# yxtay/transformer-recommenders

Measured on AMD Instinct MI355X. Metric: user-sequences/sec (train step) MovieLens-1M seq200 d128 @1/2/4/8 GPU, higher is better.
Workload: dtype bf16; 1 GPU; MovieLens-1M-shaped: 3883 items, seq_len=200, d_model=128, 4-layer causal BERT (heads=4, ffn=512), InfoNCELoss over in-batch shared negatives, AdamW; per_gpu_batch=512, global_batch=512, seq_len=200, lengths=dense, loss_heads_evaluated=all 7 + LogitsStatistics (reference training_step), parallelism=dp1, launch=eager launches

## Files before the change

### include/xfmr_hip.h

```cpp
#ifndef XFMR_HIP_H
#define XFMR_HIP_H

#include <stddef.h>
#include <stdint.h>

#ifdef __cplusplus
extern "C" {
#endif

#define XFMR_ABI_VERSION 3

enum {
  XFMR_OK = 0,
  XFMR_EINVAL = -1,
  XFMR_EUNSUPPORTED = -2,
  XFMR_EWORKSPACE = -3,
  XFMR_EHIP = -4,
  XFMR_EALIGN = -5,
  XFMR_ECOMM = -6
};

enum { XFMR_PREC_F32 = 0, XFMR_PREC_BF16 = 1 };
enum { XFMR_ATTN_CAUSAL = 0, XFMR_ATTN_BIDIRECTIONAL = 1 };
enum { XFMR_ATTN_STREAM_KEYS = 2 };
// ... 159 lines not shown
typedef struct xfmr_loss_cfg {
  int32_t train_head;
  int32_t all_heads;
  int32_t mask_false_negatives;
  int32_t mode;
  int32_t precision;
  float scale;
  float margin;
  int32_t num_hard_negatives;
  uint32_t flags;
  void* profile_grad[2];
  void* profile_log[2];
  int64_t padded_positions;
} xfmr_loss_cfg;
enum {
  XFMR_LOSS_DTOK_ZEROED = 1u
};
#define XFMR_LOSS_NSPLIT(n) (((uint32_t)(n) & 0xffu) << 8)
#define XFMR_LOSS_NSPLIT_GRAD(n) (((uint32_t)(n) & 0xffu) << 16)
#define XFMR_LOSS_NSPLIT_OF(flags) (((flags) >> 8) & 0xffu)
#define XFMR_LOSS_NSPLIT_GRAD_OF(flags) (((flags) >> 16) & 0xffu)
size_t xfmr_sampled_loss_workspace(int64_t positions, int32_t H, int64_t n_rows);
size_t xfmr_sampled_loss_workspace_cfg(const xfmr_loss_cfg* cfg, int64_t positions, int32_t H, int64_t n_rows);
int xfmr_sampled_loss(const xfmr_loss_cfg* cfg, const float* tok, const uint8_t* key_mask, const int64_t* pos_idx,
                      const int64_t* neg_idx, const float* table, const float* table_rnorm, const void* table_bf16,
                      int64_t n_rows, int64_t positions, int32_t H, float* losses, float* stats, float* d_tok, void* workspace,
                      size_t workspace_bytes, void* stream);
size_t xfmr_sampled_loss_lists_workspace(int64_t n_query, int64_t n_neg, int32_t H, int64_t n_rows);
size_t xfmr_sampled_loss_lists_workspace_cfg(const xfmr_loss_cfg* cfg, int64_t n_query, int64_t n_neg, int32_t H,
                                             int64_t n_rows);
int xfmr_sampled_loss_lists(const xfmr_loss_cfg* cfg, const float* query, const int64_t* pos_items,
// ... 126 lines not shown
```

### transformer-recommenders_amd/csrc/internal.h

```cpp
#pragma once
#include "common.h"

enum : uint32_t {
  XF_S16_A = 1u,
  XF_S16_B = 2u,
  XF_S16_C = 4u,
  XF_S16_P = 8u,
  XF_AUX_GELU_GRAD = 0x100u,
};

enum GemmOp : int32_t {
  kGemmFwdBias = 0, kGemmFwdGelu, kGemmFwdDropRes,
  kGemmLnFwd, kGemmLnFwdRe, kGemmLnFwdReDrop,
  kGemmDx, kGemmDxGelu, kGemmDxLnBwd,
  kGemmDw, kGemmDwDeferred, kGemmDwGroup,
  kGemmFfnFwd, kGemmFfnFwdRe, kGemmFfnBwd,
  kGemmOps
};
enum GemmFamily : int32_t {
  kGemmNone = 0,
  kGemmTile,
  kGemmGroup,
  kGemmRing,
  kGemmFfnFwdKernel, kGemmFfnBwdKernel,
// ... 122 lines not shown
                       float* pre, float* mean, float* rstd, uint8_t* key_mask, int32_t B, int32_t L, int32_t H,
                       float eps, float dropout_p, XfSeed seed, uint32_t site, hipStream_t stream);
int xf_embed_ln_fwd_packed_ex(const int64_t* item_idx, const float* table, int64_t n_rows, const float* pos_emb,
                              const float* type_emb, const float* gamma, const float* beta, float* out, void* out16,
                              float* pre, float* mean, float* rstd, uint8_t* key_mask, int64_t rows, const int32_t* row_pos,
                              int32_t H, float eps, float dropout_p, XfSeed seed, uint32_t site, hipStream_t stream);
int xf_embed_param_grads_packed(const float* d_pre, float* d_pos, float* d_type, const int32_t* offs, int32_t B, int32_t L,
                                int32_t H, int32_t max_pos, hipStream_t st);
int xf_encoder_plan(const xfmr_encoder_cfg* cfg, int32_t out[16]);
int xf_attn_plan(int32_t bwd, int32_t precision, int32_t s16, int32_t B, int32_t L, int32_t A, int32_t H, int32_t causal,
                 int32_t packed, int32_t stream_keys, int32_t switches, int32_t out[8]);
int xf_attn_switches();
int xf_loss_plan(int64_t T, int32_t H, int64_t n_rows, int32_t train_head, int32_t all_heads, int32_t mask_false_negatives,
                 int32_t mode, int32_t precision, int32_t num_hard_negatives, uint32_t flags, int32_t has_d_tok,
                 int32_t has_table_bf16, int32_t cus, uint64_t switches, int32_t out[40]);
uint64_t xf_loss_switches();
int xf_layernorm_bwd_impl(const float* dy, const float* x, const float* mean, const float* rstd, const float* gamma,
                          float* dx, void* d_lin, bool lin16, float* d_gamma, float* d_beta, float* d_bias,
                          int64_t rows, int32_t H, XfDropout drop_out, XfDropout drop_lin, void* partials,
                          hipStream_t st, int* blocks_out = nullptr);
}
```

### transformer-recommenders_amd/csrc/loss.hip

```cpp
#include <stdlib.h>
#include <string.h>

#include "internal.h"
#include "loss_common.h"

namespace {

constexpr int PREP = 1024;
__global__ __launch_bounds__(PREP) void prepare_count_kernel(const uint8_t* key_mask, const int64_t* pos_idx, int T,
                                                             int2* blockcnt) {
  __shared__ int sv[PREP / 64], sq[PREP / 64];
  const int i = blockIdx.x * PREP + threadIdx.x;
  const bool v = i < T && key_mask[i] != 0;
  const bool q = v && pos_idx[i] != 0;
  const int nv = __popcll(__ballot(v)), nq = __popcll(__ballot(q));
  if ((threadIdx.x & 63) == 0) { sv[threadIdx.x >> 6] = nv; sq[threadIdx.x >> 6] = nq; }
  __syncthreads();
  if (threadIdx.x == 0) {
    int a = 0, b = 0;
    for (int w = 0; w < PREP / 64; ++w) { a += sv[w]; b += sq[w]; }
    blockcnt[blockIdx.x] = make_int2(a, b);
  }
}
__global__ __launch_bounds__(PREP) void prepare_write_kernel(const uint8_t* key_mask, const int64_t* pos_idx,
// ... 824 lines not shown
struct LossPass {
  int32_t role;
  int32_t code;
  int32_t all;
  int32_t gx, gy, gz;
  int32_t nsplit;
  int32_t buf;
  int32_t image;
  int32_t finish;
  int32_t pinned;
};
struct LossPlan {
  int32_t family, hard , qprep , npass;
  LossPass pass[2];
  int32_t need_grad, nsplit, nsplit_loss, loss_buf, lse_from_grad, skip_train_head, values_only, blocks;
};
constexpr int kLossPlanInts = sizeof(LossPlan) / sizeof(int32_t);

bool loss_key_ok(int64_t rows, int64_t n_rows, int train_head, int num_hard) {
  return rows > 0 && n_rows > 0 && rows <= (1 << 30) && n_rows <= (1 << 30) && train_head >= 0 &&
         train_head < XFMR_NUM_LOSSES && num_hard >= 0;
}
constexpr int loss_main_width(bool f32, int H) {
  if (H <= 0 || (H & 31)) return 0;
  for (int w : {64, 128, 256, 384, 512})
    if (H <= w) return w;
  if (f32) return 0;
  return H <= 768 ? 768 : H <= 1024 ? 1024 : 0;
}

int loss_plan(const LossKey& k, LossPlan& lp) {
  lp = LossPlan{};
// ... 48 lines not shown
    finish = grad_pass && ns_grad == 1 && !col_parts;
    const bool lse_elsewhere = head == XFMR_LOSS_INFONCE && (grad_pass || k.all_heads == 2);
    const int lcode = loss_dma_form(H, lse_elsewhere ? -2 : -1, mask_fn, k.mode, false, k.sw.logm256);
    auto add = [&](int role, int code, int gz, int n, int buf, bool fin) {
      const bool image = !k.sw.q_fp32 && n > 1;
      lp.qprep |= image;
      lp.pass[lp.npass++] = LossPass{role, code, 0, qblocks, n, gz, n, buf, image, fin, role == kPassGrad && pinned};
    };
    if (log_pass && pinned) add(kPassLog, lcode, 1, ns, 1, false);
    if (grad_pass) add(kPassGrad, gcode, parts, ns_grad, 0, finish);
    if (log_pass && !pinned) add(kPassLog, lcode, 1, ns, grad_pass, false);
    lp.nsplit = grad_pass ? ns_grad : ns;
    lp.loss_buf = grad_pass && log_pass;
    lp.nsplit_loss = lp.loss_buf ? ns : lp.nsplit;
    lp.lse_from_grad = lp.loss_buf && lse_elsewhere;
  }
  lp.need_grad = k.d_tok && !finish;
  lp.skip_train_head = k.all_heads == 2 && !k.d_tok;
  lp.values_only = !lp.need_grad;
  const int rows = lp.values_only ? kValueRows : kCombineRows;
  lp.blocks = (int)((k.T + rows - 1) / rows);
  return XFMR_OK;
}

template <class P, int W>
void launch_main(const LossArgs& a, bool all, dim3 grid, hipStream_t st) {
  if (all) hipLaunchKernelGGL((loss_main_kernel<P, W, true>), grid, dim3(256), 0, st, a);
  else hipLaunchKernelGGL((loss_main_kernel<P, W, false>), grid, dim3(256), 0, st, a);
}
template <class P>
// ... 47 lines not shown
                     losses, stats);
  XF_LAUNCH_CHECK();
  return XFMR_OK;
}

uint64_t xf_loss_switches() { return switch_bits(loss_switches()); }
int xf_loss_plan(int64_t T, int32_t H, int64_t n_rows, int32_t train_head, int32_t all_heads, int32_t mask_false_negatives,
                 int32_t mode, int32_t precision, int32_t num_hard_negatives, uint32_t flags, int32_t has_d_tok,
                 int32_t has_table_bf16, int32_t cus, uint64_t switches, int32_t out[40]) {
  static_assert(kLossPlanInts <= 40, "xf_loss_plan's array");
  LossPlan lp;
  const int rc = loss_plan(LossKey{T, n_rows, H, train_head, all_heads, mask_false_negatives, mode, precision,
                                   num_hard_negatives, flags, has_d_tok != 0, has_table_bf16 != 0, cus,
                                   switches_of(switches)}, lp);
  memset(out, 0, 40 * sizeof(int32_t));
  memcpy(out, &lp, sizeof(lp));
  return rc;
}

size_t xfmr_sampled_loss_workspace(int64_t positions, int32_t H, int64_t n_rows) {
  if (positions <= 0 || H <= 0) return 0;
  return loss_carve(nullptr, positions, H, n_rows).total;
}
size_t xfmr_sampled_loss_workspace_cfg(const xfmr_loss_cfg* cfg, int64_t positions, int32_t H, int64_t n_rows) {
  if (!cfg || positions <= 0 || H <= 0) return 0;
  return loss_carve(cfg, positions, H, n_rows).total;
}

static int run_loss(const xfmr_loss_cfg* cfg, const float* tok, const float* table, const float* table_rnorm,
                    const void* table_bf16, int64_t n_rows, int T, int32_t H, float* losses, float* stats, float* d_tok,
                    unsigned char* ws, const Plan& p, hipStream_t st) {
// ... 21 lines not shown
    if (int rc = launch_generic(d, lp.family, lp.pass[0].code, false, dim3(lp.pass[0].gx, lp.pass[0].gy), st)) return rc;
    SelectArgs s{};
    s.dump = d.dump; s.dump_ld = p.dump_ld; s.qinfo = d.qinfo; s.counts = counts; s.neg_item = neg_item;
    s.neg_rc = a.neg_rc; s.neg_mult = a.neg_mult; s.rnorm = table_rnorm; s.qpos = qpos; s.tau = (float4*)(ws + p.off_tau);
    s.mode = cfg->mode; s.mask_fn = cfg->mask_false_negatives; s.k = cfg->num_hard_negatives; s.n_rows = n_rows;
    hipLaunchKernelGGL(hard_select_kernel, dim3((unsigned)T), dim3(256), 0, st, s);
    XF_LAUNCH_CHECK();
    a.tau = (const float4*)(ws + p.off_tau);
  }
  bool img_ready = false;
  for (int i = 0; i < lp.npass; ++i) {
    const LossPass& ps = lp.pass[i];
    LossArgs l = a;
    l.nsplit = ps.nsplit; l.part = part[ps.buf];
    if (ps.role == kPassLog) l.need_grad = 0;
    if (ps.finish) l.d_tok = d_tok;
    if (ps.pinned) { l.pin_part = part[lp.loss_buf]; l.pin_nsplit = lp.nsplit_loss; }
    if (ps.image) {
      l.qimg = (__bf16*)(ws + p.off_qimg); l.qaux = (float2*)(ws + p.off_qaux);
      if (!img_ready) {
        if (int rc = launch_qprep_h(a, (__bf16*)(ws + p.off_qimg), (float2*)(ws + p.off_qaux), H, dim3(ps.gx), st)) return rc;
        img_ready = true;
      }
    }
    void* const* ev = ps.role == kPassGrad ? cfg->profile_grad : cfg->profile_log;
    if (ev[0] && hipEventRecord((hipEvent_t)ev[0], st) != hipSuccess) return XFMR_EHIP;
    const dim3 grid(ps.gx, ps.gy, ps.gz);
    if (int rc = lp.family == kLossDma ? launch_dma_h(l, table_bf16, H, ps.code, grid, st)
                                       : launch_generic(l, lp.family, ps.code, ps.all != 0, grid, st))
      return rc;
// ... 152 lines not shown
```

### transformer-recommenders_amd/csrc/loss_common.h

```cpp
#pragma once
#include "common.h"

namespace xfl {

constexpr int BN = 64;
constexpr int QB = 128;
constexpr int REC = 16;
constexpr int LDT = BN + 4;
constexpr float kLog2e = 1.4426950408889634f;
constexpr float kLn2 = 0.6931471805599453f;
enum { R_CNTD = 0, R_M, R_L, R_NCE, R_HINGE, R_LOGI, R_CNTC, R_CONTR, R_SSUM, R_SSQ, R_SMIN, R_SMAX, R_SW,
       R_POSDOT, R_RQ, R_QQ };
constexpr int BP = 24;
constexpr int HEAD_INFONCE_MASKED = XFMR_NUM_LOSSES;
constexpr int HEAD_INFONCE_PINNED = XFMR_NUM_LOSSES + 1;
constexpr int HEAD_BPR_MASKED = XFMR_NUM_LOSSES + 2;
constexpr int HEAD_CCL_MASKED = XFMR_NUM_LOSSES + 3, HEAD_CONTR_MASKED = XFMR_NUM_LOSSES + 4;

struct LossArgs {
  const float* tok; const float* table; const float* rnorm; int64_t n_rows;
  const int* counts;
  const int* neg_item;
  const float* neg_rc;
  const float* neg_mult;
  const int* qrow; const int* qpos;
  float* part; float* partO;
  float* dump; int64_t dump_ld; float2* qinfo; const float4* tau;
  const float* pin_part;
  int pin_nsplit;
  float* d_tok;
  const __bf16* qimg; const float2* qaux;
  int T; int nsplit;
  int H;
  int train_head, mask_fn, mode, need_grad;
  float scale, margin;
};

struct RowState {
  float cnt_d, m, l, nce, hinge, logi, cnt_c, contr, ssum, ssq, smin, smax, sw;
};
struct RowConst {
  float pos_dot, cpos, chinge, sc2, rq, margin;
  int pos_item, head;
  bool mask_fn, catalog, cos_head;
  bool hard;
  float tau_d, rho_d, tau_c, rho_c;
};
template <bool ALL, int HC, int NO, bool HARD = false>
__device__ __forceinline__ void loss_epilogue_t(f32x16& s, RowState& st, f32x16 (&o)[NO], const RowConst& k,
// ... 97 lines not shown
          w = d > 0.f ? mc * rc[u] : 0.f;
      }
      if (ALL) {
        ssum = fmaf(sv, md, ssum);
        ssq = fmaf(sv * sv, md, ssq);
        smin = fminf(smin, md > 0.f ? sv : INFINITY);
        smax = fmaxf(smax, md > 0.f ? sv : -INFINITY);
      }
      sw += w;
      s[r] = w;
    }
    __builtin_amdgcn_sched_barrier(0);
  }
}

template <bool CHECK_VALID>
__device__ __forceinline__ void loss_epilogue_infonce_masked(f32x16& s, float& l, float& cnt, float pos_dot, float sc2,
                                                             float m, int pos_item, const int* nid_sb,
                                                             const float* mu_sb, int hh) {
#pragma unroll
  for (int g = 0; g < 4; ++g) {
    const int4 n4 = *reinterpret_cast<const int4*>(&nid_sb[8 * g + 4 * hh]);
    const int nn[4] = {n4.x, n4.y, n4.z, n4.w};
    const float4 m4 = *reinterpret_cast<const float4*>(&mu_sb[8 * g + 4 * hh]);
    const float mu[4] = {m4.x, m4.y, m4.z, m4.w};
#pragma unroll
    for (int u = 0; u < 4; ++u) {
      const int r = 4 * g + u;
      bool counted = (s[r] < pos_dot) & (nn[u] != pos_item);
      if (CHECK_VALID) counted &= nn[u] >= 0;
      cnt += counted ? mu[u] : 0.f;
      const float e = xf_exp2(counted ? fmaf(s[r], sc2, -m) : -INFINITY) * mu[u];
      l += e;
      s[r] = e;
    }
  }
}

__device__ __forceinline__ void loss_epilogue_bpr_masked(f32x16& s, float& logi2, float& cnt, float& sw, float pos_dot,
                                                         float chinge, int pos_item, const int* nid_sb, const float* mu_sb,
                                                         int hh) {
#pragma unroll
  for (int g = 0; g < 4; ++g) {
    const int4 n4 = *reinterpret_cast<const int4*>(&nid_sb[8 * g + 4 * hh]);
    const int nn[4] = {n4.x, n4.y, n4.z, n4.w};
    const float4 m4 = *reinterpret_cast<const float4*>(&mu_sb[8 * g + 4 * hh]);
    const float mu[4] = {m4.x, m4.y, m4.z, m4.w};
#pragma unroll
    for (int u = 0; u < 4; ++u) {
// ... 24 lines not shown
    const float4 m4 = *reinterpret_cast<const float4*>(&mu_sb[jl0]);
    const float mu[4] = {m4.x, m4.y, m4.z, m4.w};
#pragma unroll
    for (int u = 0; u < 4; ++u) {
      const int r = 4 * g + u;
      const float sc = s[r] * rc[u];
      const float mc = ((sc < kpos_c) & (nn[u] != pos_item)) ? mu[u] : 0.f;
      cnt_c += mc;
      const float dd = sc - kappa_c;
      contr_q = fmaf(fmaxf(dd, 0.f), mc, contr_q);
      s[r] = dd > 0.f ? mc * rc[u] : 0.f;
    }
  }
}

template <bool CHECK_VALID>
__device__ __forceinline__ void loss_epilogue_infonce_pinned(f32x16& s, float& l, float& cnt, float pos_dot, float sc2,
                                                             float m, int pos_item, bool catalog, const int* nid_sb,
                                                             const float* mu_sb, int hh) {
#pragma unroll
  for (int g = 0; g < 4; ++g) {
    const int4 n4 = *reinterpret_cast<const int4*>(&nid_sb[8 * g + 4 * hh]);
    const int nn[4] = {n4.x, n4.y, n4.z, n4.w};
    const float4 m4 = *reinterpret_cast<const float4*>(&mu_sb[8 * g + 4 * hh]);
    const float mu[4] = {m4.x, m4.y, m4.z, m4.w};
#pragma unroll
    for (int u = 0; u < 4; ++u) {
      const int r = 4 * g + u;
      const bool same = nn[u] == pos_item;
      const float sv = same ? pos_dot : s[r];
      bool counted = !(catalog & same);
      if (CHECK_VALID) counted &= nn[u] >= 0;
      const float w = counted ? mu[u] : 0.f;
      cnt += w;
      const float e = xf_exp2(fminf(fmaf(sv, sc2, -m), 0.f)) * w;
      l += e;
      s[r] = e;
    }
  }
}

constexpr int HEAD_LOG_MASKED = -3, HEAD_LOG_MASKED_LSE = -4;
constexpr int HEAD_LOG_UNMASKED_CATALOG = -5;
struct LogConst {
  float pos_dot, sc2, m, chinge, clog2e , kpos_c , kappa_c ;
  int pos_item;
  float kexp , k2m ;
};
template <bool CHECK_VALID, bool LSE, bool SHARE, bool MASK = true>
__device__ __forceinline__ void loss_epilogue_logging_masked(const f32x16& s, RowState& st, const LogConst& k,
                                                             const int* nid_sb, const float* rc_sb, const float* mu_sb,
                                                             int hh) {
// ... 224 lines not shown
```

### transformer-recommenders_amd/csrc/loss_dma.inc

```
#ifndef XFL_DBG
#define XFL_DBG 0
#endif
#ifndef XFL_LOGM_WAVES
#define XFL_LOGM_WAVES 3
#endif
#ifndef XFL_LOGU256_PK
#define XFL_LOGU256_PK 0
#endif
#ifndef XFL_GRAD_WAVES
#define XFL_GRAD_WAVES 2
#endif
#ifndef XFL_LOGM_LSE_WAVES
#define XFL_LOGM_LSE_WAVES 3
#endif
template <int H, int HEAD_CODE>
constexpr int loss_dma_waves() {
  return (H <= 128 && HEAD_CODE == HEAD_LOG_MASKED) ? XFL_LOGM_WAVES
         : (H <= 128 && HEAD_CODE == HEAD_LOG_MASKED_LSE) ? XFL_LOGM_LSE_WAVES
         : (H <= 128 && HEAD_CODE == HEAD_INFONCE_MASKED) ? XFL_GRAD_WAVES
         : (H <= 128 || (H <= 256 && (HEAD_CODE < 0 || loss_dma_hparts(H, HEAD_CODE) > 1))) ? 2 : 1;
}
template <int H>
__global__ __launch_bounds__(256) void loss_qprep_kernel(LossArgs a, __bf16* qimg, float2* qaux) {
  const int tid = threadIdx.x, lane = tid & 63;
  const int Nq = a.counts[1];
  const int qi = blockIdx.x * QB + (tid >> 6) * 32 + (lane & 31);
  if ((int)blockIdx.x * QB >= Nq) return;
  const bool qvalid = qi < Nq;
  const int row = qvalid ? a.qrow[qi] : 0;
  const int pos_item = qvalid ? a.qpos[qi] : -2;
  RegRows<PrecBF16, H> qreg, preg;
  float qq = qreg.load_safe_sq(a.tok + (int64_t)row * H, qvalid);
  preg.load_safe(a.table + (int64_t)(qvalid ? pos_item : 0) * H, qvalid);
  float pos_dot = qreg.dot_partial(preg);
  pos_dot += xf_half_swap(pos_dot);
  qq += xf_half_swap(qq);
  if (qvalid) {
    qreg.store_image(qimg + (int64_t)qi * H);
    if (lane < 32) qaux[qi] = make_float2(qq, pos_dot);
  }
}
template <int H>
int xf_launch_loss_qprep_t(const LossArgs& a, __bf16* qimg, float2* qaux, dim3 grid, hipStream_t st) {
  hipLaunchKernelGGL((loss_qprep_kernel<H>), dim3(grid.x), dim3(256), 0, st, a, qimg, qaux);
  XF_LAUNCH_CHECK();
  return XFMR_OK;
}

template <int H, int HEAD_CODE, bool QIMG>
__global__ __launch_bounds__(256, (loss_dma_waves<H, HEAD_CODE>())) void loss_main_dma_kernel(
    LossArgs a, const __bf16* tbf) {
  constexpr bool PINNED = HEAD_CODE == HEAD_INFONCE_PINNED;
  constexpr bool LEAN = HEAD_CODE == HEAD_INFONCE_MASKED || PINNED;
  constexpr bool LOGU = HEAD_CODE == HEAD_LOG_UNMASKED_CATALOG;
  constexpr bool LOGM = HEAD_CODE == HEAD_LOG_MASKED || HEAD_CODE == HEAD_LOG_MASKED_LSE || LOGU;
  constexpr bool BPRM = HEAD_CODE == HEAD_BPR_MASKED;
  constexpr bool COSM = HEAD_CODE == HEAD_CCL_MASKED || HEAD_CODE == HEAD_CONTR_MASKED;
  constexpr int HEAD = LEAN   ? (int)XFMR_LOSS_INFONCE
                       : BPRM ? (int)XFMR_LOSS_PAIRWISE_LOGISTIC
                       : HEAD_CODE == HEAD_CCL_MASKED   ? (int)XFMR_LOSS_ALIGNMENT_CONTRASTIVE
                       : HEAD_CODE == HEAD_CONTR_MASKED ? (int)XFMR_LOSS_CONTRASTIVE
                                                        : (LOGM ? -1 : HEAD_CODE);
  constexpr bool GRAD = HEAD >= 0;
  constexpr bool ALL = HEAD < 0;
  constexpr bool SPARSE_W = COSM || (!LEAN && !BPRM && (HEAD == (int)XFMR_LOSS_PAIRWISE_HINGE || HEAD == (int)XFMR_LOSS_CONTRASTIVE ||
                                                        HEAD == (int)XFMR_LOSS_ALIGNMENT_CONTRASTIVE));
// ... 73 lines not shown
  LogConst lk{pos_dot, sc2, pos_dot * sc2, pos_dot * (1.f - a.margin), pos_dot * (1.f - a.margin) * kLog2e,
              pos_dot * rcpos, (1.f - a.margin) * fmaxf(sqrtf(qq), 1e-8f), pos_item, 0.f, 0.f};
  lk.kexp = xf_exp2(-lk.clog2e);
  lk.k2m = xf_exp2(-lk.m);
  const float ycap = fminf(100.f, lk.clog2e + 100.f);
  LogAcc la = log_acc_zero();
  const bool log_share = LOGM && !__any(fabsf(lk.clog2e) > 64.f) &&
                         (HEAD_CODE != HEAD_LOG_MASKED_LSE || (sc2 == kLog2e && !__any(fabsf(lk.m) > 64.f)));

  const int* __restrict__ nitem = a.neg_item;
  const float* __restrict__ nrc = catalog ? a.rnorm : a.neg_rc;
  const float* __restrict__ nmul = catalog ? nullptr : a.neg_mult;
  const uint32_t tbf_lo = (uint32_t)__builtin_amdgcn_readfirstlane((int)(uint32_t)(uintptr_t)tbf);
  const uint32_t tbf_hi = (uint32_t)__builtin_amdgcn_readfirstlane((int)(uint32_t)((uintptr_t)tbf >> 32));
  const __bf16* const tbf_u = reinterpret_cast<const __bf16*>(((uint64_t)tbf_hi << 32) | (uint64_t)tbf_lo);
  auto issue_gather = [&](int lt, int buf) {
    __bf16* base = sEb + buf * TILE_ELEMS;
    int ln = lane;
    asm volatile("" : "+v"(ln));
#pragma unroll
    for (int k = 0; k < NI; ++k) {
      const int q = wid * NI + k;
      const int g = q * 64 + ln;
      const int r = g / SI::CPR, c = g % SI::CPR;
      const int id = max(sNid[lt * BN + r], 0);
      xf_glds16_raw_so(tbf_u, (uint32_t)id * (uint32_t)(2 * H) + (uint32_t)(16 * (c ^ SI::swz(r))), base + q * 512);
    }
  };

  constexpr int NFORM = LOGM ? 2 : 1;
  const int form_sel = (LOGM && !log_share) ? 1 : 0;
#pragma unroll
  for (int form = 0; form < NFORM; ++form) {
  if (form != form_sel) continue;
  for (int c0 = t_beg; c0 < t_end; c0 += CH) {
    const int c1 = min(c0 + CH, t_end);
    __syncthreads();
    for (int e = tid; e < (c1 - c0) * BN; e += 256) {
      const int j = c0 * BN + e;
      const int jc = j < N ? j : N - 1;
      const int it = catalog ? jc : nitem[jc];
      sNid[e] = (j < N || LOGM || BPRM || COSM) ? it : -1;
      sRc[e] = nrc[jc];
      sMul[e] = ((LOGM || BPRM || COSM) && j >= N) ? 0.f : (nmul ? nmul[jc] : 1.f);
    }
    __syncthreads();
    issue_gather(0, 0);
    for (int tile = c0; tile < c1; ++tile) {
      const int lt = tile - c0, buf = lt & 1;
      asm volatile("s_waitcnt vmcnt(0) lgkmcnt(0)" ::: "memory");
      __builtin_amdgcn_s_barrier();
      if (tile + 1 < c1 && !((XFL_DBG & 8) && lt > 0)) issue_gather(lt + 1, buf ^ 1);
      const __bf16* E = sEb + buf * TILE_ELEMS;
#pragma unroll 1
      for (int sb = 0; sb < BN / 32; ++sb) {
        f32x16 s;
#pragma unroll
        for (int r = 0; r < 16; ++r) s[r] = 0.f;
        if (XFL_DBG & 2) {
#pragma unroll
          for (int r = 0; r < 16; ++r) s[r] = sRc[lt * BN + sb * 32 + r] * (float)(lane + r);
        } else SI::tile_nreg(s, E, sb * 32, qreg.regs());
        if (XFL_DBG & 1) {
#pragma unroll
          for (int r = 0; r < 16; ++r) st.l += s[r];
        } else if (PINNED) {
          if ((tile + 1) * BN <= N)
            loss_epilogue_infonce_pinned<false>(s, st.l, lean_cnt, pos_dot, sc2, st.m, pos_item, catalog,
                                                &sNid[lt * BN + sb * 32], &sMul[lt * BN + sb * 32], hh);
          else
            loss_epilogue_infonce_pinned<true>(s, st.l, lean_cnt, pos_dot, sc2, st.m, pos_item, catalog,
                                               &sNid[lt * BN + sb * 32], &sMul[lt * BN + sb * 32], hh);
        } else if (LEAN) {
          if ((tile + 1) * BN <= N)
            loss_epilogue_infonce_masked<false>(s, st.l, lean_cnt, pos_dot, sc2, st.m, pos_item,
                                                &sNid[lt * BN + sb * 32], &sMul[lt * BN + sb * 32], hh);
          else
            loss_epilogue_infonce_masked<true>(s, st.l, lean_cnt, pos_dot, sc2, st.m, pos_item,
                                               &sNid[lt * BN + sb * 32], &sMul[lt * BN + sb * 32], hh);
        } else if (BPRM) {
          loss_epilogue_bpr_masked(s, st.logi, st.cnt_d, st.sw, pos_dot, pos_dot * (1.f - a.margin), pos_item,
                                   &sNid[lt * BN + sb * 32], &sMul[lt * BN + sb * 32], hh);
        } else if (COSM) {
          loss_epilogue_cos_masked(s, st.contr, st.cnt_c, lk.kpos_c, lk.kappa_c, pos_item, &sNid[lt * BN + sb * 32],
                                   &sRc[lt * BN + sb * 32], &sMul[lt * BN + sb * 32], hh);
        } else if (LOGM) {
          constexpr bool LSE = HEAD_CODE == HEAD_LOG_MASKED_LSE;
          const int* nid_sb = &sNid[lt * BN + sb * 32];
          const float* rc_sb = &sRc[lt * BN + sb * 32];
          const float* mu_sb = &sMul[lt * BN + sb * 32];
          constexpr bool PK = XFL_LOG_PK && !(LOGU && H > 128 && !XFL_LOGU256_PK);
          constexpr bool FENCE = LOGU && H > 128;
          if (PK) {
            if (form == 0) loss_epilogue_logging_masked_pk<LSE, true, !LOGU, FENCE>(s, st, la, lk, ycap, nid_sb, rc_sb, mu_sb, hh);
// ... 5 lines not shown
        } else loss_epilogue_t<ALL, HEAD>(s, st, o, kc, &sNid[lt * BN + sb * 32], &sRc[lt * BN + sb * 32],
                                          &sMul[lt * BN + sb * 32], hh);
        if (GRAD && do_grad && !(XFL_DBG & 4)) {
          bool any_w = true;
          if (SPARSE_W) {
            uint32_t bits = 0u;
#pragma unroll
            for (int r = 0; r < 16; ++r) bits |= __float_as_uint(s[r]);
            any_w = __any((bits << 1) != 0u);
          }
          if (any_w) {
#pragma unroll
            for (int i = 0; i < NO; ++i) SI::tile_xb_tr(o[i], E, hpart * NO + i, sb * 32, s);
          }
        }
      }
    }
  }

  }

  st.cnt_d += lean_cnt;
  if (BPRM) st.logi *= kLn2;
  if (COSM) st.contr *= rq;
  if (LOGM) log_acc_fold(la, st);
  if (LOGM) loss_logging_masked_finish(st, rq);
  if (HEAD == XFMR_LOSS_INFONCE) st.sw = st.l;
  const RowState ms = merge_halves(st);
  write_partial(ms, a.part + ((int64_t)split * a.T + qi) * REC, lane < 32 && qvalid && hpart == 0, pos_dot, rq, qq);
  if (GRAD && do_grad) {
    __syncthreads();
// ... 72 lines not shown
    }
    float* base = a.partO + (int64_t)split * a.T * H;
#pragma unroll
    for (int i = 0; i < NO; ++i)
      xf_store_tile_T(sScratch + wid * 32 * 33, o[i], 1.f, base + (hpart * NO + i) * 32, H, qb0 + wid * 32, Nq);
  }
}

constexpr bool loss_dma_built(int H, int code) {
  if (code <= HEAD_LOG_MASKED) return code >= HEAD_LOG_UNMASKED_CATALOG && H <= 256;
  return code != (int)XFMR_LOSS_ALIGNMENT && code <= HEAD_CONTR_MASKED;
}
template <int H, int HEAD_CODE>
int xfl_launch_code(const LossArgs& a, const __bf16* tbf, dim3 grid, hipStream_t st) {
  if constexpr (loss_dma_built(H, HEAD_CODE)) {
    if (a.qimg != nullptr) hipLaunchKernelGGL((loss_main_dma_kernel<H, HEAD_CODE, true>), grid, dim3(256), 0, st, a, tbf);
    else hipLaunchKernelGGL((loss_main_dma_kernel<H, HEAD_CODE, false>), grid, dim3(256), 0, st, a, tbf);
    XF_LAUNCH_CHECK();
    return XFMR_OK;
  }
  return XFMR_EINVAL;
}
template <int H>
int xfl_launch_form(const LossArgs& a, const __bf16* tbf, int code, dim3 grid, hipStream_t st) {
  switch (code) {
    case -1: return xfl_launch_code<H, -1>(a, tbf, grid, st);
    case -2: return xfl_launch_code<H, -2>(a, tbf, grid, st);
    case HEAD_LOG_MASKED: return xfl_launch_code<H, HEAD_LOG_MASKED>(a, tbf, grid, st);
    case HEAD_LOG_MASKED_LSE: return xfl_launch_code<H, HEAD_LOG_MASKED_LSE>(a, tbf, grid, st);
    case HEAD_LOG_UNMASKED_CATALOG: return xfl_launch_code<H, HEAD_LOG_UNMASKED_CATALOG>(a, tbf, grid, st);
// ... 15 lines not shown
```

### transformer-recommenders_amd/xfmr_rec_amd/_native.py

```python

from __future__ import annotations

import ctypes as C
import os
import pathlib

import torch

_HERE = pathlib.Path(__file__).resolve().parent
LIB_PATH = pathlib.Path(os.environ["XFMR_HIP_LIB"]) if os.environ.get("XFMR_HIP_LIB") else _HERE / "libxfmr_hip.so"

PREC_F32, PREC_BF16 = 0, 1
PRECISIONS = {"fp32": PREC_F32, "f32": PREC_F32, "bf16": PREC_BF16}
EPI_BIAS, EPI_BIAS_GELU, EPI_BIAS_DROP_RES = 0, 1, 2
NEG_SHARED, NEG_CATALOG = 0, 1
ATTN_CAUSAL, ATTN_BIDIRECTIONAL = 0, 1
ATTN_STREAM_KEYS = 2
ENC_BIDIRECTIONAL, ENC_LN_UNFUSED, ENC_FFN_UNFUSED, ENC_FFN_BWD_UNFUSED, ENC_DW_INLINE, ENC_DW_SIDE_ANY = 1, 2, 4, 8, 16, 32
ENC_DW_UNPAIRED, ENC_REDUCE_HALF_EARLY = 64, 128
LOSS_DTOK_ZEROED = 1
ABI_VERSION = 3
ECOMM = -6
NUM_LOSSES, NUM_STATS = 7, 16
RANK_NONE = 0x7FFFFFFF
MAX_RANK_CUTOFFS = 8
LOSS_IDS = {
    "AlignmentLoss": 0,
    "AlignmentContrastiveLoss": 1,
    "ContrastiveLoss": 2,
    "InfoNCELoss": 3,
    "NCELoss": 4,
    "PairwiseHingeLoss": 5,
    "PairwiseLogisticLoss": 6,
}
STAT = dict(
# ... 248 lines not shown
```

### transformer-recommenders_amd/xfmr_rec_amd/ops.py

```python

from __future__ import annotations

import ctypes as C
import dataclasses
import os

import torch

from . import _native as N

f32 = torch.float32


def _empty(shape, like: torch.Tensor, dtype=f32):
    return torch.empty(shape, dtype=dtype, device=like.device)


def _bytes(n: int, like: torch.Tensor):
    return torch.empty(max(int(n), 16), dtype=torch.uint8, device=like.device)


def selftest_mfma(device="cuda") -> list[int]:
    out = torch.full((4 + 4096,), -1, dtype=torch.int32, device=device)
    N.check(N.load().xfmr_selftest_mfma(N.ptr(out), N.stream()), "xfmr_selftest_mfma")
# ... 363 lines not shown
def sampled_loss_workspace(like, T, H, n_rows, opts=None, *, table_bf16=None, **kw):
    cfg = _entry_opts(opts, kw, True).cfg()
    return _bytes(N.load().xfmr_sampled_loss_workspace_cfg(C.byref(cfg), T, H, n_rows), like)


def sampled_loss_prepare(ws, key_mask, pos_idx, neg_idx, rnorm, n_rows, H, opts=None, *, table_bf16=None, **kw):
    cfg = _entry_opts(opts, kw, True).cfg()
    N.check(
        N.load().xfmr_sampled_loss_prepare(C.byref(cfg), N.ptr(key_mask), N.ptr(pos_idx), N.ptr(neg_idx), N.ptr(rnorm),
                                           n_rows, key_mask.numel(), H, N.ptr(ws), ws.numel(), N.stream()),
        "xfmr_sampled_loss_prepare",
    )


def sampled_loss(tok, key_mask, pos_idx, neg_idx, table, rnorm, opts=None, *, need_grad=True, table_bf16=None,
                 workspace=None, prepared=False, d_tok_zeroed=None, profile_grad=None, profile_log=None, **kw):
    o = _entry_opts(opts, kw, True)
    H = tok.shape[-1]
    T = tok.numel() // H
    lib = N.load()
    d_tok = (d_tok_zeroed if d_tok_zeroed is not None else torch.empty_like(tok)) if need_grad else None
    flags = 0
    if d_tok_zeroed is not None and need_grad:
        assert d_tok.shape == tok.shape and d_tok.dtype == tok.dtype
        flags = N.LOSS_DTOK_ZEROED
    cfg = o.cfg(flags=flags, profile_grad=profile_grad, profile_log=profile_log)
    n_rows = table.shape[0]
    losses = _empty((2 * N.NUM_LOSSES,), tok)
    stats = _empty((N.NUM_STATS,), tok)
    if workspace is None:
        assert not prepared
        nbytes = lib.xfmr_sampled_loss_workspace_cfg(C.byref(cfg), T, H, n_rows)
        ws = _bytes(nbytes, tok)
    else:
        ws, nbytes = workspace, workspace.numel()
    fn = lib.xfmr_sampled_loss_prepared if prepared else lib.xfmr_sampled_loss
    N.check(
        fn(C.byref(cfg), N.ptr(tok), N.ptr(key_mask), N.ptr(pos_idx), N.ptr(neg_idx), N.ptr(table), N.ptr(rnorm),
           N.ptr(table_bf16), n_rows, T, H, N.ptr(losses), N.ptr(stats), N.ptr(d_tok), N.ptr(ws), nbytes, N.stream()),
        "xfmr_sampled_loss_prepared" if prepared else "xfmr_sampled_loss",
# ... 372 lines not shown
```

### transformer-recommenders_amd/xfmr_rec_amd/trainer.py

```python

from __future__ import annotations

import ctypes
import math
import os
import time

import numpy as np
import torch

from . import _native as N
from . import eval_rows as E
from . import ops
from .losses import LOSS_CLASSES, LossConfig, LossType
from .models import ModelConfig, RecommenderModel
from .params import METRIC, TOP_K
from .step_plan import StepPlan, device_values, host_values, step_result

try:
    import lightning.pytorch as _lp

    _Base = _lp.LightningModule
except Exception:
    _lp = None
# ... 211 lines not shown
        side.wait_event(self._ev_embed)
        with torch.cuda.stream(side):
            for w, heads in ((ws_log, 2), (ws_grad, False)):
                ops.sampled_loss_prepare(w, key_mask, pos, neg, m.table_rnorm, n_rows, H, opts.replace(all_heads=heads))
            d_tok0 = torch.zeros_like(tok)
            self._ev_prep.record(side)
        side.wait_stream(main)
        with torch.cuda.stream(side):
            losses, stats, _ = ops.sampled_loss(
                tok.detach(), key_mask, pos, neg, m.embeddings, m.table_rnorm, opts.replace(all_heads=2), need_grad=False,
                table_bf16=m.table_bf16, workspace=ws_log, prepared=True, profile_log=profile_log
            )
        main.wait_event(self._ev_prep)
        train_loss, losses_train, _ = ops.sampled_loss_train(
            tok, key_mask, pos, neg, m.embeddings, m.table_rnorm, opts.replace(all_heads=False), table_bf16=m.table_bf16,
            workspace=ws_grad, prepared=True, d_tok_zeroed=d_tok0, profile_grad=profile_grad
        )
        for tns in (ws_log, ws_grad):
            tns.record_stream(side)
        d_tok0.record_stream(main)
        for tns in (tok, key_mask, pos, neg):
            if tns is not None:
                tns.record_stream(side)
        self._logging_pending = True
        return train_loss, losses, losses_train, stats

    def logged_values(self, out: dict) -> dict[str, float]:
        self.sync_logging()
        return host_values(out, self.config)

    @property
# ... 621 lines not shown
```

Baseline: 170,700 sequences/s.

## Skip negative counting in grad-pass InfoNCE kernel and unroll gather tiles

Adds a STATS_ELSEWHERE flag so the gradient-pass InfoNCE loss kernel can skip accumulating the negative count when the logging pass already produces it. The trainer sets this flag on its train-loss call. The change also unrolls the DMA tile loop by two with fixed buffer indices and precomputes the per-lane gather row and column offsets in registers. These cut ALU work in the hot loss kernel, but raise register pressure and may reduce occupancy.

```diff
diff --git a/include/xfmr_hip.h b/include/xfmr_hip.h
--- a/include/xfmr_hip.h
+++ b/include/xfmr_hip.h
@@ -197,7 +197,8 @@
   int64_t padded_positions;
 } xfmr_loss_cfg;
 enum {
-  XFMR_LOSS_DTOK_ZEROED = 1u
+  XFMR_LOSS_DTOK_ZEROED = 1u,
+  XFMR_LOSS_STATS_ELSEWHERE = 2u
 };
 #define XFMR_LOSS_NSPLIT(n) (((uint32_t)(n) & 0xffu) << 8)
 #define XFMR_LOSS_NSPLIT_GRAD(n) (((uint32_t)(n) & 0xffu) << 16)
diff --git a/transformer-recommenders_amd/csrc/internal.h b/transformer-recommenders_amd/csrc/internal.h
--- a/transformer-recommenders_amd/csrc/internal.h
+++ b/transformer-recommenders_amd/csrc/internal.h
@@ -160,6 +160,9 @@
 int xf_loss_plan(int64_t T, int32_t H, int64_t n_rows, int32_t train_head, int32_t all_heads, int32_t mask_false_negatives,
                  int32_t mode, int32_t precision, int32_t num_hard_negatives, uint32_t flags, int32_t has_d_tok,
                  int32_t has_table_bf16, int32_t cus, uint64_t switches, int32_t out[40]);
+int xf_loss_plan_ext(int64_t T, int32_t H, int64_t n_rows, int32_t train_head, int32_t all_heads, int32_t mask_false_negatives,
+                     int32_t mode, int32_t precision, int32_t num_hard_negatives, uint32_t flags, int32_t has_d_tok,
+                     int32_t has_table_bf16, int32_t cus, uint64_t switches, int32_t ext[8]);
 uint64_t xf_loss_switches();
 int xf_layernorm_bwd_impl(const float* dy, const float* x, const float* mean, const float* rstd, const float* gamma,
                           float* dx, void* d_lin, bool lin16, float* d_gamma, float* d_beta, float* d_bias,
diff --git a/transformer-recommenders_amd/csrc/loss.hip b/transformer-recommenders_amd/csrc/loss.hip
--- a/transformer-recommenders_amd/csrc/loss.hip
+++ b/transformer-recommenders_amd/csrc/loss.hip
@@ -862,8 +862,10 @@
   int32_t family, hard , qprep , npass;
   LossPass pass[2];
   int32_t need_grad, nsplit, nsplit_loss, loss_buf, lse_from_grad, skip_train_head, values_only, blocks;
+  int32_t grad_no_count;
 };
 constexpr int kLossPlanInts = sizeof(LossPlan) / sizeof(int32_t);
+constexpr int kLossPlanBaseInts = offsetof(LossPlan, grad_no_count) / sizeof(int32_t);
 
 bool loss_key_ok(int64_t rows, int64_t n_rows, int train_head, int num_hard) {
   return rows > 0 && n_rows > 0 && rows <= (1 << 30) && n_rows <= (1 << 30) && train_head >= 0 &&
@@ -942,6 +944,8 @@
     lp.loss_buf = grad_pass && log_pass;
     lp.nsplit_loss = lp.loss_buf ? ns : lp.nsplit;
     lp.lse_from_grad = lp.loss_buf && lse_elsewhere;
+    lp.grad_no_count = grad_pass && (gcode == HEAD_INFONCE_MASKED || gcode == HEAD_INFONCE_PINNED) &&
+                       (lp.loss_buf || (k.flags & XFMR_LOSS_STATS_ELSEWHERE) != 0);
   }
   lp.need_grad = k.d_tok && !finish;
   lp.skip_train_head = k.all_heads == 2 && !k.d_tok;
@@ -1019,7 +1023,19 @@
                                    num_hard_negatives, flags, has_d_tok != 0, has_table_bf16 != 0, cus,
                                    switches_of(switches)}, lp);
   memset(out, 0, 40 * sizeof(int32_t));
-  memcpy(out, &lp, sizeof(lp));
+  memcpy(out, &lp, kLossPlanBaseInts * sizeof(int32_t));
+  return rc;
+}
+int xf_loss_plan_ext(int64_t T, int32_t H, int64_t n_rows, int32_t train_head, int32_t all_heads, int32_t mask_false_negatives,
+                     int32_t mode, int32_t precision, int32_t num_hard_negatives, uint32_t flags, int32_t has_d_tok,
+                     int32_t has_table_bf16, int32_t cus, uint64_t switches, int32_t ext[8]) {
+  static_assert(kLossPlanInts - kLossPlanBaseInts <= 8, "xf_loss_plan_ext's array");
+  LossPlan lp;
+  const int rc = loss_plan(LossKey{T, n_rows, H, train_head, all_heads, mask_false_negatives, mode, precision,
+                                   num_hard_negatives, flags, has_d_tok != 0, has_table_bf16 != 0, cus,
+                                   switches_of(switches)}, lp);
+  memset(ext, 0, 8 * sizeof(int32_t));
+  memcpy(ext, (const int32_t*)&lp + kLossPlanBaseInts, (kLossPlanInts - kLossPlanBaseInts) * sizeof(int32_t));
   return rc;
 }
 
@@ -1071,6 +1087,7 @@
     LossArgs l = a;
     l.nsplit = ps.nsplit; l.part = part[ps.buf];
     if (ps.role == kPassLog) l.need_grad = 0;
+    else l.no_count = lp.grad_no_count;
     if (ps.finish) l.d_tok = d_tok;
     if (ps.pinned) { l.pin_part = part[lp.loss_buf]; l.pin_nsplit = lp.nsplit_loss; }
     if (ps.image) {
diff --git a/transformer-recommenders_amd/csrc/loss_common.h b/transformer-recommenders_amd/csrc/loss_common.h
--- a/transformer-recommenders_amd/csrc/loss_common.h
+++ b/transformer-recommenders_amd/csrc/loss_common.h
@@ -1,4 +1,5 @@
 #pragma once
+#include <type_traits>
 #include "common.h"
 
 namespace xfl {
@@ -33,6 +34,7 @@
   int T; int nsplit;
   int H;
   int train_head, mask_fn, mode, need_grad;
+  int no_count;
   float scale, margin;
 };
 
@@ -160,7 +162,7 @@
   }
 }
 
-template <bool CHECK_VALID>
+template <bool CHECK_VALID, bool COUNT = true, bool SPLIT_SUM = false>
 __device__ __forceinline__ void loss_epilogue_infonce_masked(f32x16& s, float& l, float& cnt, float pos_dot, float sc2,
                                                              float m, int pos_item, const int* nid_sb,
                                                              const float* mu_sb, int hh) {
@@ -175,10 +177,17 @@
       const int r = 4 * g + u;
       bool counted = (s[r] < pos_dot) & (nn[u] != pos_item);
       if (CHECK_VALID) counted &= nn[u] >= 0;
-      cnt += counted ? mu[u] : 0.f;
-      const float e = xf_exp2(counted ? fmaf(s[r], sc2, -m) : -INFINITY) * mu[u];
-      l += e;
-      s[r] = e;
+      if (COUNT) cnt += counted ? mu[u] : 0.f;
+      if constexpr (SPLIT_SUM) {
+#pragma clang fp contract(off)
+        const float e = xf_exp2(counted ? fmaf(s[r], sc2, -m) : -INFINITY) * mu[u];
+        l += e;
+        s[r] = e;
+      } else {
+        const float e = xf_exp2(counted ? fmaf(s[r], sc2, -m) : -INFINITY) * mu[u];
+        l += e;
+        s[r] = e;
+      }
     }
   }
 }
@@ -233,7 +242,7 @@
   }
 }
 
-template <bool CHECK_VALID>
+template <bool CHECK_VALID, bool COUNT = true, bool SPLIT_SUM = false>
 __device__ __forceinline__ void loss_epilogue_infonce_pinned(f32x16& s, float& l, float& cnt, float pos_dot, float sc2,
                                                              float m, int pos_item, bool catalog, const int* nid_sb,
                                                              const float* mu_sb, int hh) {
@@ -251,10 +260,17 @@
       bool counted = !(catalog & same);
       if (CHECK_VALID) counted &= nn[u] >= 0;
       const float w = counted ? mu[u] : 0.f;
-      cnt += w;
-      const float e = xf_exp2(fminf(fmaf(sv, sc2, -m), 0.f)) * w;
-      l += e;
-      s[r] = e;
+      if (COUNT) cnt += w;
+      if constexpr (SPLIT_SUM) {
+#pragma clang fp contract(off)
+        const float e = xf_exp2(fminf(fmaf(sv, sc2, -m), 0.f)) * w;
+        l += e;
+        s[r] = e;
+      } else {
+        const float e = xf_exp2(fminf(fmaf(sv, sc2, -m), 0.f)) * w;
+        l += e;
+        s[r] = e;
+      }
     }
   }
 }
diff --git a/transformer-recommenders_amd/csrc/loss_dma.inc b/transformer-recommenders_amd/csrc/loss_dma.inc
--- a/transformer-recommenders_amd/csrc/loss_dma.inc
+++ b/transformer-recommenders_amd/csrc/loss_dma.inc
@@ -19,6 +19,20 @@
          : (H <= 128 && HEAD_CODE == HEAD_LOG_MASKED_LSE) ? XFL_LOGM_LSE_WAVES
          : (H <= 128 && HEAD_CODE == HEAD_INFONCE_MASKED) ? XFL_GRAD_WAVES
          : (H <= 128 || (H <= 256 && (HEAD_CODE < 0 || loss_dma_hparts(H, HEAD_CODE) > 1))) ? 2 : 1;
+}
+#ifndef XFL_TILE_UNROLL
+#define XFL_TILE_UNROLL 1
+#endif
+#ifndef XFL_GATHER_RESIDENT
+#define XFL_GATHER_RESIDENT 1
+#endif
+template <int H, int HEAD_CODE>
+constexpr bool loss_dma_unrolled() {
+  return XFL_TILE_UNROLL != 0 && H <= 256 && (HEAD_CODE == HEAD_INFONCE_MASKED || HEAD_CODE == HEAD_INFONCE_PINNED);
+}
+template <int H, int HEAD_CODE>
+constexpr bool loss_dma_gather_resident() {
+  return XFL_GATHER_RESIDENT != 0 && loss_dma_waves<H, HEAD_CODE>() <= 2 && H <= 256 && HEAD_CODE > (int)XFMR_LOSS_INFONCE;
 }
 template <int H>
 __global__ __launch_bounds__(256) void loss_qprep_kernel(LossArgs a, __bf16* qimg, float2* qaux) {
@@ -47,9 +61,12 @@
   return XFMR_OK;
 }
 
-template <int H, int HEAD_CODE, bool QIMG>
+template <int H, int HEAD_CODE, bool QIMG, bool COUNT = true>
 __global__ __launch_bounds__(256, (loss_dma_waves<H, HEAD_CODE>())) void loss_main_dma_kernel(
     LossArgs a, const __bf16* tbf) {
+  static_assert(COUNT || HEAD_CODE == HEAD_INFONCE_MASKED || HEAD_CODE == HEAD_INFONCE_PINNED, "every other head needs its count");
+  constexpr bool UNROLLED = loss_dma_unrolled<H, HEAD_CODE>();
+  constexpr bool SPLIT_SUM = H > 128;
   constexpr bool PINNED = HEAD_CODE == HEAD_INFONCE_PINNED;
   constexpr bool LEAN = HEAD_CODE == HEAD_INFONCE_MASKED || PINNED;
   constexpr bool LOGU = HEAD_CODE == HEAD_LOG_UNMASKED_CATALOG;
@@ -153,17 +170,37 @@
   const uint32_t tbf_lo = (uint32_t)__builtin_amdgcn_readfirstlane((int)(uint32_t)(uintptr_t)tbf);
   const uint32_t tbf_hi = (uint32_t)__builtin_amdgcn_readfirstlane((int)(uint32_t)((uintptr_t)tbf >> 32));
   const __bf16* const tbf_u = reinterpret_cast<const __bf16*>(((uint64_t)tbf_hi << 32) | (uint64_t)tbf_lo);
+  constexpr bool GRES = loss_dma_gather_resident<H, HEAD_CODE>();
+  uint32_t g_row[GRES ? NI : 1], g_cb[GRES ? NI : 1];
+  if constexpr (GRES) {
+#pragma unroll
+    for (int k = 0; k < NI; ++k) {
+      const uint32_t g = (uint32_t)((wid * NI + k) * 64) + (uint32_t)lane;
+      const uint32_t r = g / (uint32_t)SI::CPR, c = g % (uint32_t)SI::CPR;
+      g_row[k] = r;
+      g_cb[k] = 16u * (c ^ (uint32_t)SI::swz((int)r));
+      asm volatile("" : "+v"(g_row[k]), "+v"(g_cb[k]));
+    }
+  }
   auto issue_gather = [&](int lt, int buf) {
     __bf16* base = sEb + buf * TILE_ELEMS;
-    int ln = lane;
-    asm volatile("" : "+v"(ln));
-#pragma unroll
-    for (int k = 0; k < NI; ++k) {
-      const int q = wid * NI + k;
-      const int g = q * 64 + ln;
-      const int r = g / SI::CPR, c = g % SI::CPR;
-      const int id = max(sNid[lt * BN + r], 0);
-      xf_glds16_raw_so(tbf_u, (uint32_t)id * (uint32_t)(2 * H) + (uint32_t)(16 * (c ^ SI::swz(r))), base + q * 512);
+    if constexpr (GRES) {
+#pragma unroll
+      for (int k = 0; k < NI; ++k) {
+        const int id = max(sNid[lt * BN + (int)g_row[k]], 0);
+        xf_glds16_raw_so(tbf_u, (uint32_t)id * (uint32_t)(2 * H) + g_cb[k], base + (wid * NI + k) * 512);
+      }
+    } else {
+      uint32_t ln = (uint32_t)lane;
+      asm volatile("" : "+v"(ln));
+#pragma unroll
+      for (int k = 0; k < NI; ++k) {
+        const int q = wid * NI + k;
+        const uint32_t g = (uint32_t)(q * 64) + ln;
+        const uint32_t r = g / (uint32_t)SI::CPR, c = g % (uint32_t)SI::CPR;
+        const int id = max(sNid[lt * BN + (int)r], 0);
+        xf_glds16_raw_so(tbf_u, (uint32_t)id * (uint32_t)(2 * H) + 16u * (c ^ (uint32_t)SI::swz((int)r)), base + q * 512);
+      }
     }
   };
 
@@ -185,13 +222,19 @@
     }
     __syncthreads();
     issue_gather(0, 0);
-    for (int tile = c0; tile < c1; ++tile) {
-      const int lt = tile - c0, buf = lt & 1;
+    constexpr int TU = UNROLLED ? 2 : 1, SBU = UNROLLED ? 2 : 1;
+    static_assert(BN / 32 == 2, "two sub-blocks per tile");
+    for (int tile0 = c0; tile0 < c1; tile0 += TU) {
+#pragma unroll
+    for (int tu = 0; tu < TU; ++tu) {
+      const int tile = tile0 + tu;
+      if (TU > 1 && tile >= c1) break;
+      const int lt = tile - c0, buf = UNROLLED ? tu : (lt & 1);
       asm volatile("s_waitcnt vmcnt(0) lgkmcnt(0)" ::: "memory");
       __builtin_amdgcn_s_barrier();
       if (tile + 1 < c1 && !((XFL_DBG & 8) && lt > 0)) issue_gather(lt + 1, buf ^ 1);
       const __bf16* E = sEb + buf * TILE_ELEMS;
-#pragma unroll 1
+#pragma unroll SBU
       for (int sb = 0; sb < BN / 32; ++sb) {
         f32x16 s;
 #pragma unroll
@@ -205,18 +248,18 @@
           for (int r = 0; r < 16; ++r) st.l += s[r];
         } else if (PINNED) {
           if ((tile + 1) * BN <= N)
-            loss_epilogue_infonce_pinned<false>(s, st.l, lean_cnt, pos_dot, sc2, st.m, pos_item, catalog,
-                                                &sNid[lt * BN + sb * 32], &sMul[lt * BN + sb * 32], hh);
+            loss_epilogue_infonce_pinned<false, COUNT, SPLIT_SUM>(s, st.l, lean_cnt, pos_dot, sc2, st.m, pos_item, catalog,
+                                                       &sNid[lt * BN + sb * 32], &sMul[lt * BN + sb * 32], hh);
           else
-            loss_epilogue_infonce_pinned<true>(s, st.l, lean_cnt, pos_dot, sc2, st.m, pos_item, catalog,
-                                               &sNid[lt * BN + sb * 32], &sMul[lt * BN + sb * 32], hh);
+            loss_epilogue_infonce_pinned<true, COUNT, SPLIT_SUM>(s, st.l, lean_cnt, pos_dot, sc2, st.m, pos_item, catalog,
+                                                      &sNid[lt * BN + sb * 32], &sMul[lt * BN + sb * 32], hh);
         } else if (LEAN) {
           if ((tile + 1) * BN <= N)
-            loss_epilogue_infonce_masked<false>(s, st.l, lean_cnt, pos_dot, sc2, st.m, pos_item,
-                                                &sNid[lt * BN + sb * 32], &sMul[lt * BN + sb * 32], hh);
+            loss_epilogue_infonce_masked<false, COUNT, SPLIT_SUM>(s, st.l, lean_cnt, pos_dot, sc2, st.m, pos_item,
+                                                       &sNid[lt * BN + sb * 32], &sMul[lt * BN + sb * 32], hh);
           else
-            loss_epilogue_infonce_masked<true>(s, st.l, lean_cnt, pos_dot, sc2, st.m, pos_item,
-                                               &sNid[lt * BN + sb * 32], &sMul[lt * BN + sb * 32], hh);
+            loss_epilogue_infonce_masked<true, COUNT, SPLIT_SUM>(s, st.l, lean_cnt, pos_dot, sc2, st.m, pos_item,
+                                                      &sNid[lt * BN + sb * 32], &sMul[lt * BN + sb * 32], hh);
         } else if (BPRM) {
           loss_epilogue_bpr_masked(s, st.logi, st.cnt_d, st.sw, pos_dot, pos_dot * (1.f - a.margin), pos_item,
                                    &sNid[lt * BN + sb * 32], &sMul[lt * BN + sb * 32], hh);
@@ -252,7 +295,9 @@
             for (int i = 0; i < NO; ++i) SI::tile_xb_tr(o[i], E, hpart * NO + i, sb * 32, s);
           }
         }
-      }
+        if (UNROLLED) __builtin_amdgcn_sched_barrier(0);
+      }
+    }
     }
   }
 
@@ -355,6 +400,15 @@
 template <int H, int HEAD_CODE>
 int xfl_launch_code(const LossArgs& a, const __bf16* tbf, dim3 grid, hipStream_t st) {
   if constexpr (loss_dma_built(H, HEAD_CODE)) {
+    constexpr bool LEAN_NCE = HEAD_CODE == HEAD_INFONCE_MASKED || HEAD_CODE == HEAD_INFONCE_PINNED;
+    if constexpr (LEAN_NCE) {
+      if (a.no_count) {
+        if (a.qimg != nullptr) hipLaunchKernelGGL((loss_main_dma_kernel<H, HEAD_CODE, true, false>), grid, dim3(256), 0, st, a, tbf);
+        else hipLaunchKernelGGL((loss_main_dma_kernel<H, HEAD_CODE, false, false>), grid, dim3(256), 0, st, a, tbf);
+        XF_LAUNCH_CHECK();
+        return XFMR_OK;
+      }
+    } else if (a.no_count) return XFMR_EINVAL;
     if (a.qimg != nullptr) hipLaunchKernelGGL((loss_main_dma_kernel<H, HEAD_CODE, true>), grid, dim3(256), 0, st, a, tbf);
     else hipLaunchKernelGGL((loss_main_dma_kernel<H, HEAD_CODE, false>), grid, dim3(256), 0, st, a, tbf);
     XF_LAUNCH_CHECK();
diff --git a/transformer-recommenders_amd/xfmr_rec_amd/_native.py b/transformer-recommenders_amd/xfmr_rec_amd/_native.py
--- a/transformer-recommenders_amd/xfmr_rec_amd/_native.py
+++ b/transformer-recommenders_amd/xfmr_rec_amd/_native.py
@@ -19,6 +19,7 @@
 ENC_BIDIRECTIONAL, ENC_LN_UNFUSED, ENC_FFN_UNFUSED, ENC_FFN_BWD_UNFUSED, ENC_DW_INLINE, ENC_DW_SIDE_ANY = 1, 2, 4, 8, 16, 32
 ENC_DW_UNPAIRED, ENC_REDUCE_HALF_EARLY = 64, 128
 LOSS_DTOK_ZEROED = 1
+LOSS_STATS_ELSEWHERE = 2
 ABI_VERSION = 3
 ECOMM = -6
 NUM_LOSSES, NUM_STATS = 7, 16
diff --git a/transformer-recommenders_amd/xfmr_rec_amd/ops.py b/transformer-recommenders_amd/xfmr_rec_amd/ops.py
--- a/transformer-recommenders_amd/xfmr_rec_amd/ops.py
+++ b/transformer-recommenders_amd/xfmr_rec_amd/ops.py
@@ -401,7 +401,8 @@
 
 
 def sampled_loss(tok, key_mask, pos_idx, neg_idx, table, rnorm, opts=None, *, need_grad=True, table_bf16=None,
-                 workspace=None, prepared=False, d_tok_zeroed=None, profile_grad=None, profile_log=None, **kw):
+                 workspace=None, prepared=False, d_tok_zeroed=None, stats_elsewhere=False, profile_grad=None,
+                 profile_log=None, **kw):
     o = _entry_opts(opts, kw, True)
     H = tok.shape[-1]
     T = tok.numel() // H
@@ -411,6 +412,8 @@
     if d_tok_zeroed is not None and need_grad:
         assert d_tok.shape == tok.shape and d_tok.dtype == tok.dtype
         flags = N.LOSS_DTOK_ZEROED
+    if stats_elsewhere:
+        flags |= N.LOSS_STATS_ELSEWHERE
     cfg = o.cfg(flags=flags, profile_grad=profile_grad, profile_log=profile_log)
     n_rows = table.shape[0]
     losses = _empty((2 * N.NUM_LOSSES,), tok)
diff --git a/transformer-recommenders_amd/xfmr_rec_amd/trainer.py b/transformer-recommenders_amd/xfmr_rec_amd/trainer.py
--- a/transformer-recommenders_amd/xfmr_rec_amd/trainer.py
+++ b/transformer-recommenders_amd/xfmr_rec_amd/trainer.py
@@ -249,7 +249,7 @@
         main.wait_event(self._ev_prep)
         train_loss, losses_train, _ = ops.sampled_loss_train(
             tok, key_mask, pos, neg, m.embeddings, m.table_rnorm, opts.replace(all_heads=False), table_bf16=m.table_bf16,
-            workspace=ws_grad, prepared=True, d_tok_zeroed=d_tok0, profile_grad=profile_grad
+            workspace=ws_grad, prepared=True, d_tok_zeroed=d_tok0, stats_elsewhere=True, profile_grad=profile_grad
         )
         for tns in (ws_log, ws_grad):
             tns.record_stream(side)
```

Result: faster. 172,600 sequences/s (median of 6 runs) (+1.1%).
